# alexklwong/calibrated-backprojection-network

Hardware: AMD Instinct MI355X
Metric: depth-completion frames/sec at 352x1216 (higher is better)
Workload: dtype f32; 1 GPU; KITTI 352x1216, batch 32/GPU, fp32, full KBNet forward in HIP, random xavier weights; frames_per_gpu=32, global_batch=32, height=352, width=1216, n_ranks_seen=1, collective_backend=nccl, gathered_frames=32, launch=HIP graph replay, 2 concurrent sub-batch branch(es)

## Files before the change

### calibrated-backprojection-network_amd/_lib.py

```python

from __future__ import annotations

import ctypes as C
import os

import torch

HERE = os.path.dirname(os.path.abspath(__file__))
LIB_PATH = os.environ.get("KBN_LIB_PATH") or os.path.join(HERE, "libkbnet_hip.so")

KBN_OK = 0
KBN_ERR_INVALID_ARGUMENT, KBN_ERR_UNSUPPORTED, KBN_ERR_WORKSPACE, KBN_ERR_LAUNCH = -1, -2, -3, -4
KBN_SRC_TENSOR, KBN_SRC_COORDS, KBN_SRC_XYZ, KBN_SRC_PAIR = 0, 1, 2, 3
KBN_ACT_ELU, KBN_ACT_SIGMOID = 1, 2
KBN_RESIZE_NONE, KBN_RESIZE_NEAREST = 0, 1
KBN_MAX_SRC = 3
KBN_ADAM_TABLE_CAPACITY, KBN_ADAM_PASS_ELEMENTS = 48, 524288
KBN_MULTI_COPY_TABLE_CAPACITY, KBN_MULTI_COPY_PASS_ELEMENTS = 48, 524288
KBN_AUGMENT_ROLE_IMAGE, KBN_AUGMENT_ROLE_RANGE, KBN_AUGMENT_ROLE_VALIDITY = 0, 1, 2
KBN_AUGMENT_RANGE_0_255, KBN_AUGMENT_RANGE_0_1, KBN_AUGMENT_RANGE_M1_1 = 0, 1, 2
KBN_AUGMENT_NOISE_NONE, KBN_AUGMENT_NOISE_GAUSSIAN, KBN_AUGMENT_NOISE_UNIFORM = 0, 1, 2
KBN_AUGMENT_STAGE_SELECT, KBN_AUGMENT_STAGE_APPLY = 1, 2
KBN_AUGMENT_MAX_FRAMES, KBN_AUGMENT_WORKSPACE_RECORD_BYTES = 512, 16
KBN_UNPACK_TRAIN_MAX_FRAMES = 64
# ... 202 lines not shown
    "kbn_add_act_backward": (_I, [_P, _P, _P, _L, _I, _F, _P]),
    "kbn_resize_nearest_forward": (_I, [_P, _L, _P, _L, _I, _I, _I, _I, _I, _I, _P]),
    "kbn_resize_nearest_backward": (_I, [_P, _L, _P, _L, _I, _I, _I, _I, _I, _I, _P]),
    "kbn_kb_xyz_backward": (_I, [_P, _L, _P, _L, _P, _L, _P, _L, _I, _I, _I, _I, _F, _P]),
    "kbn_depth_map_backward": (_I, [_P, _P, _P, _P, _L, _F, _P]),
    "kbn_depth_head_forward": (_I, [_P, _P, _P, _P, _I, _I, _I, _I, _F, _F, _P]),
    "kbn_conv_head_forward": (_I, [_P, _L, _P, _P, _P, _P, _I, _I, _I, _I, _I, _F, _F, _F, _P]),
    "kbn_conv_tail_packed_weight_bytes": (C.c_size_t, [_I]),
    "kbn_conv_tail_pack_weight": (_I, [_P, _P, _I, _P]),
    "kbn_conv_tail_forward": (_I, [_P, _L, _P, _P, _P, _P, _I, _I, _I, _I, _I, _F, _F, _F, _P]),
    "kbn_conv_tail_forward_pair": (_I, [_P, _L, _P, _P, _P, _P, _P, _I, _I, _I, _I, _I, _F, _F, _F, _P]),
    "kbn_absmax_frames": (_I, [_P, _L, _I, _L, _P, _P]),
    "kbn_conv3x3_split_packed_weight_bytes": (C.c_size_t, [_I, _I, _I]),
    "kbn_conv3x3_split_pack_weight": (_I, [_P, _P, _I, _I, _I, _P]),
    "kbn_conv3x3_split_forward": (_I, [C.POINTER(ConvSrc), _I, _P, _P, _L, _I, _I, _I, _I, _I, _I, _I, _F, _P, _P, _L, _P, _P]),
    "kbn_conv3x3_split_forward_ksplit": (_I, [C.POINTER(ConvSrc), _I, _P, _P, _L, _I, _I, _I, _I, _I, _I, _I, _F, _P, _I, _P, _P]),
    "kbn_conv1x1s2_split_packed_weight_bytes": (C.c_size_t, [_I, _I, _I]),
    "kbn_conv1x1s2_split_pack_weight": (_I, [_P, _P, _I, _I, _I, _P]),
    "kbn_conv1x1s2_split_forward": (_I, [C.POINTER(ConvSrc), _I, _P, _P, _L, _P, _L, _I, _I, _I, _I, _I, _I, _F, _P, _P]),
    "kbn_kb_xyz_s2_forward": (_I, [_P, _L, _I, _I, _I, _P, _P, _I, _F, _P, _L, _I, _P]),
    "kbn_adam_step": (_I, [C.POINTER(AdamTensor), _I, _P]),
    "kbn_multi_tensor_scale_copy": (_I, [C.POINTER(CopyTensor), _I, _F, _P]),
    "kbn_augment_workspace_bytes": (C.c_size_t, [C.POINTER(AugmentTensor), _I, _I, _I, _I]),
    "kbn_augment_forward": (_I, [C.POINTER(AugmentTensor), _I, C.c_char_p, _I, _I, _I, _P, _P, C.c_size_t, _I, _I, _F, C.c_ulonglong, C.c_uint, _I, _P]),
    "kbn_augment_forward_at": (_I, [C.POINTER(AugmentTensor), _I, C.c_char_p, _I, _I, _I, _P, _P, C.c_size_t, _I, _I, _F, C.c_ulonglong, C.c_uint, C.c_uint, _I, _P]),
    "kbn_summary_panel_forward": (_I, [C.POINTER(SummaryRow), _I, _I, _I, _I, _F, _P, _P]),
    "kbn_summary_colorize_forward": (_I, [_P, _L, _L, _L, _I, _I, _I, _I, _P, _P]),
    "kbn_png_info": (_I, [_P, C.c_size_t, _P, _P, _P, _P]),
    "kbn_png_decode": (_I, [_P, C.c_size_t, _P, C.c_size_t]),
    "kbn_png_decode_batch": (_I, [_P, _P, _P, _P, _I, _I, _P]),
# ... 60 lines not shown
```

### calibrated-backprojection-network_amd/csrc/abi.hip

```cpp
#include <stdlib.h>
#include <string.h>

#include "kbn_common.h"

namespace kbn {

KnobValue g_knobs[KNOB_COUNT];

static const char* const kKnobNames[KNOB_COUNT] = {
    "KBN_DEBUG", "KBN_FORCE_MW", "KBN_FORCE_TWB", "KBN_EPI_LDS", "KBN_NO_WINO",
    "KBN_NO_UP2X9", "KBN_NO_UP2X3", "KBN_WINO_RT",
    "KBN_NO_KB_PAIR", "KBN_NO_KB_DEPTH_FUSION", "KBN_PAIR_CAND", "KBN_S2D_DEBUG", "KBN_AUTOTUNE",
    "KBN_NO_HEAD_FUSION", "KBN_NO_SPLIT", "KBN_NO_OVERLAP", "KBN_NO_PAIR", "KBN_NO_PAIR_MID", "KBN_NO_PAIR_ENC",
    "KBN_NO_PAIR_TAIL", "KBN_NO_DEPTH_FRONT_FUSION", "KBN_FP16_ONE_TERM", "KBN_DEPTH_FRONT_FUSION", "KBN_NO_FRONT_NEXT"};

void tune_reload_env();

static void load_knobs() {
    for (int k = 0; k < KNOB_COUNT; ++k) {
        const char* v = getenv(kKnobNames[k]);
        g_knobs[k].set = (v && *v) ? 1 : 0;
        int val = 0;
        if (v && *v) {
            char* end = nullptr;
            const long parsed = strtol(v, &end, 10);
            val = (end == v) ? 1 : (int)parsed;
        }
        g_knobs[k].value = val;
    }
// ... 51 lines not shown
```

### calibrated-backprojection-network_amd/csrc/conv_split.hip

```cpp
#include "split_common.h"

#ifndef KBN_SPLIT_PRIO
#define KBN_SPLIT_PRIO 0
#endif

namespace kbn {

__global__ void split_scale_kernel(const float* __restrict__ w, float* __restrict__ inv_scale, int OC, int per_filter) {
    const int oc = blockIdx.x;
    __shared__ float red[256];
    float m = 0.f;
    if (oc < OC)
        for (int i = threadIdx.x; i < per_filter; i += 256) m = fmaxf(m, fabsf(w[(long long)oc * per_filter + i]));
    red[threadIdx.x] = m;
    __syncthreads();
    for (int s = 128; s > 0; s >>= 1) {
        if (threadIdx.x < s) red[threadIdx.x] = fmaxf(red[threadIdx.x], red[threadIdx.x + s]);
        __syncthreads();
    }
    if (threadIdx.x == 0) {
        int ex = SP_WEXP;
        if (red[0] > 0.f && red[0] < 3.0e38f) (void)frexpf(red[0], &ex);
        int e = SP_WEXP - ex;
        e = e > 100 ? 100 : (e < -100 ? -100 : e);
// ... 176 lines not shown
                       reinterpret_cast<float*>(static_cast<unsigned char*>(packed) + bytes - l1_bytes), out_channels, in_channels, 9);
    if (mode == 3) upconv_split_pack(weight, inv, wp, out_channels, in_channels, ocpad, total, tr, (hipStream_t)stream);
    else split_pack_launch(weight, inv, wp, out_channels, in_channels * 9, in_channels, nt, total, 9, in_channels, 0, (hipStream_t)stream);
    KBN_CHECK_LAUNCH();
    return KBN_OK;
}

int kbn_absmax_frames(const float* x, long long batch_stride, int n, long long per_frame, unsigned* slots, kbn_stream_t stream) {
    return kbn::absmax_frames_launch(x, batch_stride, n, per_frame, slots, (hipStream_t)stream);
}

static int conv3x3_split_impl(const kbn_conv_src* srcs, int n_src, const void* packed_weight, float* out,
                              long long out_batch_stride, int n, int out_channels, int height, int width, int mode,
                              int act_exponent, int apply_activation, float negative_slope, unsigned* out_absmax,
                              void* pair_out, long long pair_out_batch_stride, float* pair_out_scale, int ksplit, float* workspace,
                              kbn_stream_t stream) {
    using namespace kbn;
    if (act_exponent < -60 || act_exponent > 60) return KBN_ERR_INVALID_ARGUMENT;
    if (!srcs || n_src < 1 || n_src > 2 || !packed_weight || (!out && !pair_out) || n < 1 || out_channels < 1 || height < 1 || width < 1)
        return KBN_ERR_INVALID_ARGUMENT;
    if (mode == 4) mode = 3;
    if (mode < 0 || mode > 3) return KBN_ERR_INVALID_ARGUMENT;
    if (knob(KNOB_NO_SPLIT)) return KBN_ERR_UNSUPPORTED;
    const bool vec4 = pair_out || !((width & 3) || (reinterpret_cast<uintptr_t>(out) & 15) || (out_batch_stride & 3));
    if (!vec4 && (mode == 1 || mode == 3)) return KBN_ERR_UNSUPPORTED;
    if ((mode == 1 || mode == 3) && (n_src != 1 || (height & 1) || (width & 1))) return KBN_ERR_UNSUPPORTED;
    SplitConvParams p{};
    int cin = 0;
    for (int s = 0; s < n_src; ++s) {
        const kbn_conv_src& a = srcs[s];
        const bool pair = a.kind == KBN_SRC_PAIR;
// ... 33 lines not shown
    p.nTilesN = ceil_div(out_channels, ntf);
    p.inv_scale = static_cast<const float*>(packed_weight);
    p.wp = reinterpret_cast<const _Float16*>(p.inv_scale + p.nTilesN * ntf);
    p.l1 = reinterpret_cast<const float*>(static_cast<const unsigned char*>(packed_weight) +
                                          kbn_conv3x3_split_packed_weight_bytes(out_channels, cin, mode) - (size_t)(cin / SP_CK) * 4);
    if (pair_out) {
        const bool narrow = mode == 3 && uf_narrow(out_channels, cin);
        const bool kernel_ok = (mode == 0) || (mode == 3 && ntf == U64_NT && !uf_narrow(out_channels, cin)) ||
                               (mode == 2 && n_src == 1) || narrow;
        if (!kernel_ok || (!narrow && (out_channels & 7))) return KBN_ERR_UNSUPPORTED;
        const int pair_channels = narrow ? U16_NT : out_channels;
        if (!p.amax[0] || (n_src > 1 && !p.amax[1]) || !pair_out_scale || (reinterpret_cast<uintptr_t>(pair_out) & 15) ||
            (pair_out_batch_stride & 7) || pair_out_batch_stride < (long long)(pair_channels / 8) * 2 * pair_plane_halves(height, width))
            return KBN_ERR_INVALID_ARGUMENT;
        p.pair_out = static_cast<_Float16*>(pair_out); p.pair_out_bstride = pair_out_batch_stride; p.pair_out_scale = pair_out_scale;
    }
    if (p.pair_src && mode == 3 && !(ntf == U64_NT || uf_narrow(out_channels, cin))) return KBN_ERR_UNSUPPORTED;
    if (p.pair_src && mode == 3 && uf_narrow(out_channels, cin) && (srcs[0].channels % U16_CK)) return KBN_ERR_UNSUPPORTED;
    p.out = out; p.out_bstride = out_batch_stride;
    p.N = n; p.OC = out_channels; p.Cin = cin; p.H = height; p.W = width;
    p.tilesX = ceil_div(width, SP_TW); p.tilesY = ceil_div(height, mode == 2 ? SpGeom<2>::TH : SpGeom<0>::TH);
    if (mode == 3) { p.tilesX = ceil_div(p.sW, 32); p.tilesY = ceil_div(p.sH, 16); }
    const long long blocks = (long long)p.tilesX * p.tilesY * n * p.nTilesN;
    if (blocks > 0x7fffffffLL) return KBN_ERR_UNSUPPORTED;
    p.nblocks = (int)blocks;
    p.act = apply_activation ? 1 : 0; p.slope = negative_slope;
    p.prescale = ldexpf(1.f, act_exponent); p.unscale = ldexpf(1.f, -act_exponent);
    p.vec4 = vec4 ? 1 : 0;
    p.ksplit = 1;
    if (ksplit > 1) {
// ... 53 lines not shown
        }, p.pair_src != nullptr, p.pair_out != nullptr, one_term);
    }
    if (rc != KBN_OK) return rc;
    KBN_CHECK_LAUNCH();
    return KBN_OK;
}

int kbn_conv3x3_split_forward(const kbn_conv_src* srcs, int n_src, const void* packed_weight, float* out,
                              long long out_batch_stride, int n, int out_channels, int height, int width, int mode,
                              int act_exponent, int apply_activation, float negative_slope, unsigned* out_absmax,
                              void* pair_out, long long pair_out_batch_stride, float* pair_out_scale, kbn_stream_t stream) {
    return conv3x3_split_impl(srcs, n_src, packed_weight, out, out_batch_stride, n, out_channels, height, width, mode, act_exponent,
                              apply_activation, negative_slope, out_absmax, pair_out, pair_out_batch_stride, pair_out_scale, 1, nullptr, stream);
}

int kbn_conv3x3_split_forward_ksplit(const kbn_conv_src* srcs, int n_src, const void* packed_weight, float* out,
                                     long long out_batch_stride, int n, int out_channels, int height, int width, int mode,
                                     int act_exponent, int apply_activation, float negative_slope, unsigned* out_absmax,
                                     int ksplit, float* workspace, kbn_stream_t stream) {
    if (ksplit < 1) return KBN_ERR_INVALID_ARGUMENT;
    return conv3x3_split_impl(srcs, n_src, packed_weight, out, out_batch_stride, n, out_channels, height, width, mode, act_exponent,
                              apply_activation, negative_slope, out_absmax, nullptr, 0, nullptr, ksplit, workspace, stream);
}

}
```

### calibrated-backprojection-network_amd/csrc/kbn_common.h

```cpp
#pragma once

#include <hip/hip_runtime.h>
#include <stdint.h>

#include <atomic>
#include <type_traits>

#include "../../include/kbnet_hip.h"

#define KBN_CHECK_LAUNCH()                                   \
    do {                                                     \
        hipError_t e__ = hipGetLastError();                  \
        if (e__ != hipSuccess) return KBN_ERR_LAUNCH;        \
    } while (0)

namespace kbn {

typedef float f32x4 __attribute__((ext_vector_type(4)));
typedef float f32x2 __attribute__((ext_vector_type(2)));

__host__ __device__ inline int ceil_div(int a, int b) { return (a + b - 1) / b; }
__host__ __device__ inline int round_up(int a, int b) { return ceil_div(a, b) * b; }
inline bool layer_shape_ok(int out_channels, int in_channels, int kernel_size) {
    return out_channels >= 1 && in_channels >= 1 && kernel_size >= 1 && kernel_size <= 7 && out_channels <= KBN_MAX_CHANNELS &&
// ... 55 lines not shown
template <class F>
int flag_dispatch(F&& f) { return f(); }
template <class F, class... Flags>
int flag_dispatch(F&& f, bool flag, Flags... rest) {
    auto bind = [&](auto c) { return flag_dispatch([&](auto... more) { return f(c, more...); }, rest...); };
    return flag ? bind(std::true_type{}) : bind(std::false_type{});
}
int device_cu_count();

enum Knob {
    KNOB_DEBUG, KNOB_FORCE_MW, KNOB_FORCE_TWB, KNOB_EPI_LDS, KNOB_NO_WINO,
    KNOB_NO_UP2X9, KNOB_NO_UP2X3, KNOB_WINO_RT,
    KNOB_NO_KB_PAIR, KNOB_NO_KB_DEPTH_FUSION, KNOB_PAIR_CAND, KNOB_S2D_DEBUG, KNOB_AUTOTUNE,
    KNOB_NO_HEAD_FUSION, KNOB_NO_SPLIT,
    KNOB_NO_OVERLAP, KNOB_NO_PAIR, KNOB_NO_PAIR_MID, KNOB_NO_PAIR_ENC, KNOB_NO_PAIR_TAIL, KNOB_NO_DEPTH_FRONT_FUSION,
    KNOB_FP16_ONE_TERM, KNOB_DEPTH_FRONT_FUSION, KNOB_NO_FRONT_NEXT, KNOB_COUNT
};
struct KnobValue { int set, value; };
extern KnobValue g_knobs[KNOB_COUNT];
inline int knob(Knob k) { return g_knobs[k].value; }
inline bool knob_set(Knob k) { return g_knobs[k].set != 0; }

__device__ __forceinline__ int xcd_remap(int bid, int nblocks) {
    const int NX = 8;
    int xcd = bid % NX, idx = bid / NX;
    int q = nblocks / NX, r = nblocks % NX;
    int start = (xcd < r) ? xcd * (q + 1) : r * (q + 1) + (xcd - r) * q;
    return start + idx;
}

__device__ __forceinline__ int nearest_src_index(int dst, int in_size, int out_size) {
// ... 14 lines not shown
```

### calibrated-backprojection-network_amd/csrc/split_common.h

```cpp

#pragma once
#include "conv_common.h"

#include <type_traits>

#ifndef KBN_SPLIT_STRAIGHT
#define KBN_SPLIT_STRAIGHT 1
#endif

namespace kbn {

typedef _Float16 sph8 __attribute__((ext_vector_type(8)));
typedef _Float16 sph2 __attribute__((ext_vector_type(2)));
typedef float spf16 __attribute__((ext_vector_type(16)));
typedef float spf4 __attribute__((ext_vector_type(4)));
typedef _Float16 sph4 __attribute__((ext_vector_type(4)));

constexpr int SP_TW = 32, SP_CK = 16, SP_TH = 16, SP_THREADS = 512;
constexpr int SP_WEXP = 13;

template <int MODE>
struct SpGeom {
    static constexpr bool S2 = MODE == 2;
    static constexpr int TH = S2 ? 8 : SP_TH;
// ... 19 lines not shown
    int tilesX, tilesY, nTilesN, nblocks;
    int act;
    float slope;
    int vec4;
    float prescale;
    float unscale;
    const unsigned* amax[2];
    unsigned* out_amax;
    const _Float16* pair_src;
    long long pair_src_bstride;
    const float* pair_src_scale;
    _Float16* pair_out;
    long long pair_out_bstride;
    float* pair_out_scale;
    const float* l1;
    int tp_x0, tp_tilesY, tp_nblocks;
    int sub0;
    const float* xyz;
    long long xyz_bstride;
    const float* wxyz;
    int ksplit;
    long long ks_stride;
};

__device__ __forceinline__ void sp_split8(const float (&v)[8], float prescale, sph8& h1, sph8& h2) {
    const float prescale_hi = prescale * 2048.f;
#pragma unroll
    for (int k = 0; k < 8; k += 2) {
        const f32x2 a = {v[k], v[k + 1]};
        const sph2 c1 = __builtin_convertvector(a * prescale, sph2);
// ... 23 lines not shown
}


__device__ __forceinline__ float sp_scale_of_bound(float bound) {
    int k = 14 + 127 - (int)(__float_as_uint(bound) >> 23 & 255u);
    k = k > 100 ? 100 : (k < -100 ? -100 : k);
    return __uint_as_float((unsigned)(127 + k) << 23);
}
__device__ __forceinline__ float sp_pair_out_scale(const SplitConvParams& p, int n) {
    const int nchunks = p.Cin / SP_CK, n0 = p.nsrc > 1 ? p.srcC[0] / SP_CK : nchunks;
    float w0 = 0.f, w1 = 0.f;
    for (int c = 0; c < n0; ++c) w0 += p.l1[c];
    for (int c = n0; c < nchunks; ++c) w1 += p.l1[c];
    float bound = __uint_as_float(p.amax[0][n]) * w0;
    if (p.nsrc > 1) bound += __uint_as_float(p.amax[1][n]) * w1;
    return sp_scale_of_bound(bound);
}
__device__ __forceinline__ void sp_act_scale_of(const SplitConvParams& p, int s, int n, float& prescale, float& unscale) {
    prescale = p.prescale;
    unscale = p.unscale;
    if (p.amax[s]) {
        int k = 14 + 127 - (int)(p.amax[s][n] >> 23);
        k = k > 100 ? 100 : (k < -100 ? -100 : k);
        prescale = __uint_as_float((unsigned)(127 + k) << 23);
        unscale = __uint_as_float((unsigned)(127 - k) << 23);
    }
}
typedef unsigned spu2 __attribute__((ext_vector_type(2)));
typedef unsigned spu4 __attribute__((ext_vector_type(4)));
__device__ __forceinline__ spu4 sp_pair_exchange(const sph4& a, const sph4& b) {
// ... 48 lines not shown
```

### calibrated-backprojection-network_amd/modules.py

```python

from __future__ import annotations

import os
from typing import List, Optional

import torch

from . import _lib, ops, optim
from ._lib import KbnError
from .config import KBNetConfig


def activation_func(activation_fn: str):
    if "linear" in activation_fn:
        return None
    if "leaky_relu" in activation_fn:
        return torch.nn.LeakyReLU(negative_slope=0.20, inplace=True)
    if "relu" in activation_fn:
        return torch.nn.ReLU()
    if "elu" in activation_fn:
        return torch.nn.ELU()
    if "sigmoid" in activation_fn:
        return torch.nn.Sigmoid()
    raise ValueError("Unsupported activation function: {}".format(activation_fn))
# ... 55 lines not shown
        if self._blob is not None:
            self.get(*self._args[0], **self._args[1])


def packed_blobs(model):
    return [v for top in model.modules() for sub in top.modules() for v in vars(sub).values() if isinstance(v, _PackedBlob)]


def data_gradient_blob(layer, weight):
    blob = layer.__dict__.get("_packed_bwd_data")
    if blob is None:
        blob = layer._packed_bwd_data = _PackedBlob(ops.pack_conv2d_data_gradient_weight)
    return blob.get(weight, stride=layer.stride)


def _run_split(layer, weight, srcs, n, h, w, out=None, up2x=False, out_absmax=None, stats=None, pair_out=False, transposed=False):
    kinds_ok = all((s.kind == _lib.KBN_SRC_TENSOR or (i == 0 and s.kind == _lib.KBN_SRC_PAIR)) and s.channels % 16 == 0
                   for i, s in enumerate(srcs))
    if (not layer.split or layer.kernel_size != 3 or (up2x and w % 4) or len(srcs) > 2 or (up2x and layer.stride != 1)
            or not kinds_ok or (pair_out and layer._post is not None)):
        return None
    narrow_up = up2x and layer.split_narrow_up and layer.out_channels <= 16 and layer.in_channels % 32 == 0
    if layer.out_channels < 48 and not narrow_up:
        return None
    dev = weight.device
    srcs = Conv2d._with_slots(srcs, n, dev, stats)
    if pair_out:
        if stats is None or (layer.out_channels % 8 and not narrow_up) or (layer.stride != 1 and up2x):
            return None
        out = ops.PairTensor(n, 16 if narrow_up else layer.out_channels, h, w, dev, stats)
        if layer.stride == 2:
            out.with_sub()
        if out_absmax is not None:
            out.absmax = out_absmax
    elif out is None:
        out = torch.empty((n, layer.out_channels, h, w), device=dev, dtype=torch.float32)
    packed = layer._split_blob(up2x)
    ks = 1
    if getattr(layer, "latency", 0) and not pair_out and all(s.kind == _lib.KBN_SRC_TENSOR for s in srcs):
        ks = ops.ksplit_for(sum(s.channels for s in srcs), layer.out_channels, h, w, layer.stride, up2x=up2x, frames=layer.latency)
    kw = dict(up2x=up2x, negative_slope=layer._slope, stride=layer.stride, folded_up2x=up2x, out_absmax=None if layer._post else out_absmax,
              transposed=transposed)
    res = ops.conv3x3_split(srcs, packed, n, layer.out_channels, h, w, out, ksplit=ks, **kw) if ks > 1 else None
    if res is None:
        res = ops.conv3x3_split(srcs, packed, n, layer.out_channels, h, w, out, **kw)
    return res if res is None else _finish(layer, res, out_absmax)


class Conv2d(torch.nn.Module):

    def __init__(self, in_channels, out_channels, kernel_size=3, stride=1,
                 weight_initializer="kaiming_uniform",
                 activation_func=torch.nn.LeakyReLU(negative_slope=0.10, inplace=True),
                 use_batch_norm=False, use_instance_norm=False):
        super().__init__()
        if use_batch_norm or use_instance_norm:
            raise ValueError("normalisation layers are not part of the KBNet inference path")
# ... 19 lines not shown
    def _with_slots(srcs, n, dev, stats):
        for s in srcs:
            if s.kind == _lib.KBN_SRC_TENSOR and (not s.absmax or (stats is not None and not stats.usable(s.absmax))):
                if stats is None:
                    stats = ops.ActStats(n, dev, capacity=len(srcs))
                slot = stats.measure(s._keep[0])
                s.absmax = slot.data_ptr()
                s._keep = (s._keep[0], slot)
        return srcs

    def _split_blob(self, up2x):
        if up2x:
            return self._packed_split_up.get(self.conv.weight, folded_up2x=True)
        return self._packed_split.get(self.conv.weight, stride=self.stride)

    def run_split(self, srcs, n, h, w, out=None, up2x=False, out_absmax=None, stats=None, pair_out=False):
        return _run_split(self, self.conv.weight, srcs, n, h, w, out, up2x, out_absmax, stats, pair_out)

    def split_fused_qualifies(self, ci, cf):
        return (self.split and self.kernel_size == 1 and self.stride == 2 and ci % 16 == 0 and cf % 16 == 0
                and self.out_channels >= self.split_fused_min_filters and self.in_channels == ci + 3 + cf)

    def run_split_fused(self, image, fused, xyz, n, h, w, out, amax_image=None, amax_fused=None, out_absmax=None, stats=None):
        ci, cf = image.shape[1], (0 if fused is None else fused.shape[1])
        if not self.split_fused_qualifies(ci, cf):
            return None
        if isinstance(image, ops.PairTensor):
            if image.sub is None or fused is None:
                return None
            image, amax_image = image.sub, image.absmax
        srcs = [ops.tensor_src(image, "image", amax_image)] + ([] if fused is None else [ops.tensor_src(fused, "fused", amax_fused)])
        srcs = self._with_slots(srcs, n, image.device, stats)
# ... 424 lines not shown
                parts = [ops.s2d_pyramid(x, mins[i:i + 8], []) for i in range(0, len(mins), 8)]
                parts += [ops.s2d_pyramid(x, [], maxs[i:i + 8]) for i in range(0, len(maxs), 8)]
                y = torch.cat(parts, dim=1)
            for conv in self.pool_convs:
                y = conv.run([ops.tensor_src(y, "pool")], n, h, w)
            return self.conv.run([ops.tensor_src(y, "pool"), ops.tensor_src(x, "x")], n, h, w)
        return ops.s2d_forward(x, [c.conv.weight for c in self.pool_convs], self.conv.conv.weight,
                               self.min_pool_sizes, self.max_pool_sizes, self._slope)


class KBNetEncoder(torch.nn.Module):

    pair_chain = _KnobSwitch("KBN_NO_PAIR", "KBN_NO_PAIR_ENC")
    fuse_s2d = _KnobSwitch("KBN_NO_DEPTH_FRONT_FUSION", enable="KBN_DEPTH_FRONT_FUSION")
    front_next = _KnobSwitch("KBN_NO_FRONT_NEXT")

    def __init__(self, input_channels_image=3, input_channels_depth=1,
                 n_filters_image=[48, 96, 192, 384, 384], n_filters_depth=[16, 32, 64, 128, 128],
                 n_filters_fused=[48, 96, 192, 384, 384], n_convolutions_image=[1, 1, 1, 1, 1],
                 n_convolutions_depth=[1, 1, 1, 1, 1], n_convolutions_fused=[1, 1, 1, 1, 1],
                 resolutions_backprojection=[0, 1, 2], weight_initializer="kaiming_uniform",
                 activation_func="leaky_relu"):
        super().__init__()
        for lst in (n_convolutions_image, n_convolutions_depth, n_convolutions_fused, n_filters_image,
                    n_filters_depth, n_filters_fused):
            assert len(lst) == 5
        if 0 not in resolutions_backprojection:
            raise ValueError("resolution 0 must use calibrated backprojection (undefined in the reference otherwise)")
        self.resolutions_backprojection = list(resolutions_backprojection)
        act = globals()["activation_func"](activation_func)
# ... 99 lines not shown
            raise KbnError("kb1_front declined a problem kbn_kb1_front_query accepted")
        return skip, out_image, out_depth, out_fused, a_img, a_skip, nxt_info

    def _image_splitk(self, level, h, w):
        blk = getattr(self, f"calibrated_backprojection{level + 1}", None)
        if blk is None:
            return False
        ci = blk.conv_image.conv_block[0]
        frames = getattr(ci, "latency", 0)
        return bool(frames) and ops.ksplit_for(ci.in_channels, ci.out_channels, (h + 1) // 2, (w + 1) // 2, 2, frames=frames) > 1

    def forward(self, image, depth, intrinsics):
        latent, skips, _, _ = self.encode(image, depth, intrinsics)
        return latent, skips

    def encode(self, image, depth, intrinsics, stats=None, s2d=None):
        fi, fd, ff = self._f
        n, _, h0, w0 = image.shape
        if stats is None:
            stats = ops.ActStats(n, image.device)
        dev = image.device
        image = image if _dense(image) else image.contiguous()
        if depth is not None:
            depth = depth if _dense(depth) else depth.contiguous()
        intrinsics = intrinsics.contiguous()

        kinv = ops.intrinsics_inverse(intrinsics, 1.0, 1.0)
        h, w = h0, w0
        h1, w1 = (h0 + 1) // 2, (w0 + 1) // 2
        sx, sy = w1 / w0, h1 / h0
        kinv1_box = []
# ... 65 lines not shown
            amax_skips.append(a_skip)
            h, w = oh, ow
        oh, ow = (h + 1) // 2, (w + 1) // 2
        amax_latent = stats.new()
        if 4 in self.resolutions_backprojection:
            if 3 not in self.resolutions_backprojection:
                raise AttributeError("'KBNetEncoder' object has no attribute 'calibrated_backprojection4'")
            blk = self.calibrated_backprojection4
            if isinstance(conv_image, ops.PairTensor):
                conv_image, amax_image = conv_image.float(), None
            latent = torch.empty((n, blk.n_filter_fused + blk.n_filter_depth, oh, ow), device=dev, dtype=torch.float32)
            blk.run(conv_image, conv_depth, kinv1_get(), conv_fused, None, latent[:, blk.n_filter_fused:], latent[:, :blk.n_filter_fused],
                    amax_image=amax_image, amax_fused=amax_skip if conv_fused is not None else None, out_amax_image=stats.new(),
                    out_amax_skip=amax_latent, stats=stats, need_image=not self.skip_unused_image)
            return latent, skips, amax_latent, amax_skips
        latent = torch.empty((n, fi[4] + fd[4], oh, ow), device=dev, dtype=torch.float32)
        src, a_src = (conv_fused, amax_skip) if conv_fused is not None else (conv_image, amax_image)
        branch = _SideBranch(dev)
        self.conv5_image.run([ops.tensor_src(src, "image", a_src)], n, h, w, out=latent[:, :fi[4]],
                             out_absmax=amax_latent, stats=stats)
        with branch:
            self.conv5_depth.run([ops.tensor_src(conv_depth, "depth", amax_skip)], n, h, w, out=latent[:, fi[4]:],
                                 out_absmax=amax_latent, stats=stats)
        return latent, skips, amax_latent, amax_skips


class MultiScaleDecoder(torch.nn.Module):

    pair_chain = _KnobSwitch("KBN_NO_PAIR")
    pair_tail = _KnobSwitch("KBN_NO_PAIR_TAIL")

    def __init__(self, input_channels=256, output_channels=1, n_resolution=1,
# ... 3 lines not shown
        super().__init__()
        if n_resolution != 1 or output_func != "linear" or len(n_filters) != 5 or output_channels != 1:
            raise ValueError("implemented for KBNet's decoder: 5 levels, n_resolution=1, linear 1-channel output")
        if use_batch_norm or use_instance_norm:
            raise ValueError("normalisation layers are not part of the KBNet inference path")
        self.n_resolution = n_resolution
        self.output_func = output_func
        act = globals()["activation_func"](activation_func)
        cin = input_channels
        for i, name in enumerate(("deconv4", "deconv3", "deconv2", "deconv1", "deconv0")):
            setattr(self, name, DecoderBlock(cin, n_skips[i], n_filters[i], weight_initializer, act,
                                             deconv_type=deconv_type))
            cin = n_filters[i]
        self.output0 = Conv2d(n_filters[4], output_channels, 3, 1, weight_initializer, None)
        self._packed_tail = _PackedBlob(ops.pack_conv_tail_weight)

    def features(self, x, skips, shape):
        stats = ops.ActStats(x.shape[0], x.device)
        x, amax = self.features_level1(x, skips, stats=stats)
        return self.deconv0(x, None, shape=tuple(shape)[-2:], amax_x=amax, stats=stats)

    def features_level1(self, x, skips, amax_x=None, amax_skips=None, stats=None, allow_pair=False):
        if stats is None:
            stats = ops.ActStats(x.shape[0], x.device)
        amax_skips = amax_skips if amax_skips is not None else [None] * 4
        amax = amax_x
        for blk, i in ((self.deconv4, 3), (self.deconv3, 2), (self.deconv2, 1), (self.deconv1, 0)):
            a_out = stats.new()
            y = None
            if not isinstance(x, ops.PairTensor) and blk.latency_splitk(x.shape[2], x.shape[3]):
# ... 234 lines not shown
        if return_inner:
            raise KbnError("KBNetModel.forward: return_inner exists on the recorded path only (trainable=True, grad mode on, a parameter "
                           "that requires grad): the fused forward never materialises most activations")
        return self._forward_fused(image, sparse_depth, validity_map_depth, intrinsics, return_logits, out)

    @torch.no_grad()
    def _forward_fused(self, image, sparse_depth, validity_map_depth, intrinsics, return_logits=False, out=None):
        if out is not None and return_logits:
            raise KbnError("out= and return_logits are mutually exclusive")
        input_depth = paired_planes(sparse_depth, validity_map_depth)
        if input_depth is None:
            input_depth = torch.cat([sparse_depth, validity_map_depth], dim=1)
        shape = input_depth.shape[-2:]
        stats = ops.ActStats(image.shape[0], image.device)
        latent, skips, amax_latent, amax_skips = self.encoder.encode(image, None, intrinsics, stats,
                                                                     s2d=(self.sparse_to_dense_pool, input_depth.contiguous()))
        return self.decoder.depth(latent, skips, shape, self.min_predict_depth, self.max_predict_depth,
                                  return_logits=return_logits, out=out, amax_x=amax_latent, amax_skips=amax_skips, stats=stats)

    def set_latency_mode(self, enabled: bool = True, frames: int = 1):
        frames = int(frames) if enabled else 0
        if enabled and frames < 1:
            raise KbnError("set_latency_mode: frames must be at least 1")
        for top in self.modules():
            for m in top.modules():
                if isinstance(m, (Conv2d, TransposeConv2d)):
                    m.latency = frames
        self.latency_mode = frames
        return self

    def capture(self, image, sparse_depth, validity_map_depth, intrinsics, branches=None, tune=True, outputs=1, split_graphs=False):
# ... 85 lines not shown
```

### calibrated-backprojection-network_amd/ops.py

```python

from __future__ import annotations

import contextlib
import ctypes as C
import functools
import struct
from typing import List, Optional, Sequence

import torch

from . import _lib
from ._lib import ConvSrc, KbnError, check


def _stream() -> int:
    return torch.cuda.current_stream().cuda_stream


def _on_tensor_device(fn):
    @functools.wraps(fn)
    def wrapper(*args, **kwargs):
        idx = None
        for a in list(args) + list(kwargs.values()):
            if isinstance(a, torch.Tensor) and a.is_cuda:
# ... 300 lines not shown
            PairTensor.LOG.append(self)
        self.shape = (n, channels, height, width)
        self.data = torch.empty((n, channels // 8, 2, height * width + 1, 8), device=device, dtype=torch.float16)
        self.scale = torch.empty(n, device=device, dtype=torch.float32)
        self.absmax = stats.new()
        self.sub: Optional[torch.Tensor] = None

    @property
    def device(self):
        return self.data.device

    def with_sub(self) -> "PairTensor":
        n, c, h, w = self.shape
        self.sub = torch.empty((n, c, (h + 1) // 2, (w + 1) // 2), device=self.data.device, dtype=torch.float32)
        return self

    def window_slack_log2(self) -> torch.Tensor:
        amax = slot_values(self.absmax).double().clamp_min(1e-300)
        return 15.0 - torch.log2(amax * self.scale.double())

    def float(self) -> torch.Tensor:
        n, c, h, w = self.shape
        v = self.data[:, :, 0, :h * w].double() + self.data[:, :, 1, :h * w].double() / 2048.0
        v = v / self.scale.double().view(n, 1, 1, 1)
        return v.permute(0, 1, 3, 2).reshape(n, c, h, w).float()


def pair_src(t: PairTensor, name="src") -> ConvSrc:
    n, c, h, w = t.shape
    s = ConvSrc()
# ... 318 lines not shown
            px = sh * 32 * (sw // 32) + -(-sh // 2) * 32
        else:
            px = sh * (-(-sw // seg) * seg)
        return 3 * 2.0 * n * px * cin * 16 * (-(-out_channels // nblk) * nblk)
    if stride == 1 and width >= 32 and 1 <= width % 32 <= 16:
        px = height * 32 * (width // 32) + -(-height // 2) * 32
    else:
        px = height * (-(-width // 32) * 32)
    return 3 * 2.0 * n * px * cin * 9 * (-(-out_channels // 32) * 32)


@_on_tensor_device
def conv3x3_split(srcs: List[ConvSrc], packed_weight: torch.Tensor, n: int, out_channels: int, height: int, width: int,
                  out: torch.Tensor, up2x: bool = False, negative_slope: Optional[float] = 0.2, stride: int = 1,
                  act_exponent: int = -6, folded_up2x: bool = False, out_absmax: Optional[torch.Tensor] = None,
                  transposed: bool = False, ksplit: int = 1):
    if transposed and not (up2x and folded_up2x):
        raise KbnError("conv3x3_split: transposed goes with up2x and folded_up2x")
    if up2x and stride != 1:
        raise KbnError("conv3x3_split: up2x and stride 2 are mutually exclusive")
    lib = _lib.load()
    arr = (ConvSrc * len(srcs))(*srcs)
    pair = isinstance(out, PairTensor)
    if pair:
        optr, obs = (None, 0) if (out.sub is None or stride != 2) else _planes(out.sub, "out.sub")
        if out_absmax is None:
            out_absmax = out.absmax
    else:
        optr, obs = _planes(out, "out")
    want = (n, 16 if (pair and up2x and folded_up2x and out_channels <= 16) else out_channels, height, width)
    if tuple(out.shape) != want:
        raise KbnError(f"out has shape {tuple(out.shape)}, expected {want}")
    cin = sum(s.channels for s in srcs)
    flops = 2.0 * n * height * width * cin * 9 * out_channels / (4 if transposed else 1)
    mode = (4 if transposed else (3 if folded_up2x else 1)) if up2x else (2 if stride == 2 else 0)
    if ksplit > 1:
        if pair or mode == 1:
            raise KbnError("conv3x3_split: ksplit goes with the plain / stride-2 / folded up-conv forms and an fp32 output")
        ws = torch.empty((ksplit, n, out_channels, height, width), device=out.device, dtype=torch.float32)
        done = _launched("kbn_conv3x3_split_forward_ksplit", ("conv_split", "", "conv_split_s2", "conv_split_upfold", "conv_split_upfold")[mode], flops,
                         lambda: lib.kbn_conv3x3_split_forward_ksplit(arr, len(srcs), packed_weight.data_ptr(), optr, obs, n, out_channels, height, width,
                                                                      mode, max(-60, min(60, int(act_exponent))), *_act_args(negative_slope),
                                                                      _slot_ptr(out_absmax, n), int(ksplit), ws.data_ptr(), _stream()),
                         executed=conv3x3_split_executed_flops(n, cin, out_channels, height, width, stride, up2x and folded_up2x),
                         pipe="fp16", nbytes=_src_bytes(srcs, n) + 4.0 * n * height * width * out_channels * (1 + 2 * ksplit))
        return out if done else None
    if not _launched("kbn_conv3x3_split_forward", ("conv_split", "conv_split_up", "conv_split_s2", "conv_split_upfold", "conv_split_upfold")[mode], flops,
                     lambda: lib.kbn_conv3x3_split_forward(arr, len(srcs), packed_weight.data_ptr(), optr, obs, n,
                                                           out_channels, height, width,
                                                           mode, max(-60, min(60, int(act_exponent))),
# ... 2119 lines not shown
```

### include/kbnet_hip.h

```cpp
#ifndef KBNET_HIP_H
#define KBNET_HIP_H

#include <stddef.h>

#ifdef __cplusplus
extern "C" {
#endif

#define KBN_ABI_VERSION 11

typedef void* kbn_stream_t;

typedef enum kbn_status {
    KBN_OK = 0,
    KBN_ERR_INVALID_ARGUMENT = -1,
    KBN_ERR_UNSUPPORTED = -2,
    KBN_ERR_WORKSPACE = -3,
    KBN_ERR_LAUNCH = -4
} kbn_status;

int kbn_version(void);
const char* kbn_status_string(int status);

void kbn_reload_env(void);
// ... 82 lines not shown

int kbn_deconv2x_pack_weight(const float* weight, float* packed, int out_channels, int in_channels,
                             kbn_stream_t stream);
int kbn_deconv2x_forward(const float* src, long long src_batch_stride, const float* packed_weight,
                         float* out, long long out_batch_stride, int n, int in_channels,
                         int out_channels, int src_height, int src_width, int apply_activation,
                         float negative_slope, unsigned* out_absmax, kbn_stream_t stream);

size_t kbn_conv3x3_split_packed_weight_bytes(int out_channels, int in_channels, int mode);
int kbn_conv3x3_split_pack_weight(const float* weight, void* packed, int out_channels, int in_channels, int mode,
                                  kbn_stream_t stream);
int kbn_conv3x3_split_forward(const kbn_conv_src* srcs, int n_src, const void* packed_weight, float* out,
                              long long out_batch_stride, int n, int out_channels, int height, int width, int mode,
                              int act_exponent, int apply_activation, float negative_slope, unsigned* out_absmax,
                              void* pair_out, long long pair_out_batch_stride, float* pair_out_scale, kbn_stream_t stream);
int kbn_conv3x3_split_forward_ksplit(const kbn_conv_src* srcs, int n_src, const void* packed_weight, float* out,
                                     long long out_batch_stride, int n, int out_channels, int height, int width, int mode,
                                     int act_exponent, int apply_activation, float negative_slope, unsigned* out_absmax,
                                     int ksplit, float* workspace, kbn_stream_t stream);

size_t kbn_conv1x1s2_split_packed_weight_bytes(int out_channels, int tensor_channels, int has_xyz);
int kbn_conv1x1s2_split_pack_weight(const float* weight, void* packed, int out_channels, int in_channels, int xyz_offset,
                                    kbn_stream_t stream);
int kbn_conv1x1s2_split_forward(const kbn_conv_src* srcs, int n_src, const void* packed_weight, const float* xyz,
                                long long xyz_batch_stride, float* out, long long out_batch_stride, int n, int out_channels,
                                int height, int width, int act_exponent, int apply_activation, float negative_slope,
                                unsigned* out_absmax, kbn_stream_t stream);
int kbn_kb_xyz_s2_forward(const float* depth, long long depth_batch_stride, int depth_channels, int height, int width,
                          const float* proj_weight, const float* kinv, int apply_activation, float negative_slope, float* xyz,
                          long long xyz_batch_stride, int n, kbn_stream_t stream);
// ... 360 lines not shown
```

Baseline: 3069 frames/s.

## Emit encoder latent as shared-scale fp16 pair tensor from both conv5 branches

The conv5 image and depth convolutions now write straight into one fp16 PairTensor latent, each into its own channel range. To make that possible they share one quantisation scale: each kernel's bound also takes in the peer branch's weight L1 norms and activation absmax. This drops the fp32 latent write and the later conversion into pair form for the decoder's first up-convolution. In exchange the scale computation grows, precision may drop for the branch with the smaller range, and many eligibility checks gate the path.

```diff
diff --git a/calibrated-backprojection-network_amd/_lib.py b/calibrated-backprojection-network_amd/_lib.py
--- a/calibrated-backprojection-network_amd/_lib.py
+++ b/calibrated-backprojection-network_amd/_lib.py
@@ -240,6 +240,8 @@
     "kbn_conv3x3_split_packed_weight_bytes": (C.c_size_t, [_I, _I, _I]),
     "kbn_conv3x3_split_pack_weight": (_I, [_P, _P, _I, _I, _I, _P]),
     "kbn_conv3x3_split_forward": (_I, [C.POINTER(ConvSrc), _I, _P, _P, _L, _I, _I, _I, _I, _I, _I, _I, _F, _P, _P, _L, _P, _P]),
+    "kbn_conv3x3_split_forward_shared": (_I, [C.POINTER(ConvSrc), _I, _P, _P, _L, _I, _I, _I, _I, _I, _I, _I, _F, _P, _P, _L, _P,
+                                               _P, _I, _I, _I, _P, _P]),
     "kbn_conv3x3_split_forward_ksplit": (_I, [C.POINTER(ConvSrc), _I, _P, _P, _L, _I, _I, _I, _I, _I, _I, _I, _F, _P, _I, _P, _P]),
     "kbn_conv1x1s2_split_packed_weight_bytes": (C.c_size_t, [_I, _I, _I]),
     "kbn_conv1x1s2_split_pack_weight": (_I, [_P, _P, _I, _I, _I, _P]),
diff --git a/calibrated-backprojection-network_amd/csrc/abi.hip b/calibrated-backprojection-network_amd/csrc/abi.hip
--- a/calibrated-backprojection-network_amd/csrc/abi.hip
+++ b/calibrated-backprojection-network_amd/csrc/abi.hip
@@ -12,7 +12,8 @@
     "KBN_NO_UP2X9", "KBN_NO_UP2X3", "KBN_WINO_RT",
     "KBN_NO_KB_PAIR", "KBN_NO_KB_DEPTH_FUSION", "KBN_PAIR_CAND", "KBN_S2D_DEBUG", "KBN_AUTOTUNE",
     "KBN_NO_HEAD_FUSION", "KBN_NO_SPLIT", "KBN_NO_OVERLAP", "KBN_NO_PAIR", "KBN_NO_PAIR_MID", "KBN_NO_PAIR_ENC",
-    "KBN_NO_PAIR_TAIL", "KBN_NO_DEPTH_FRONT_FUSION", "KBN_FP16_ONE_TERM", "KBN_DEPTH_FRONT_FUSION", "KBN_NO_FRONT_NEXT"};
+    "KBN_NO_PAIR_TAIL", "KBN_NO_DEPTH_FRONT_FUSION", "KBN_FP16_ONE_TERM", "KBN_DEPTH_FRONT_FUSION", "KBN_NO_FRONT_NEXT",
+    "KBN_NO_PAIR_SKIP"};
 
 void tune_reload_env();
 
diff --git a/calibrated-backprojection-network_amd/csrc/conv_split.hip b/calibrated-backprojection-network_amd/csrc/conv_split.hip
--- a/calibrated-backprojection-network_amd/csrc/conv_split.hip
+++ b/calibrated-backprojection-network_amd/csrc/conv_split.hip
@@ -214,7 +214,7 @@
                               long long out_batch_stride, int n, int out_channels, int height, int width, int mode,
                               int act_exponent, int apply_activation, float negative_slope, unsigned* out_absmax,
                               void* pair_out, long long pair_out_batch_stride, float* pair_out_scale, int ksplit, float* workspace,
-                              kbn_stream_t stream) {
+                              kbn_stream_t stream, const float* peer_l1 = nullptr, int peer_chunks = 0, const unsigned* peer_absmax = nullptr) {
     using namespace kbn;
     if (act_exponent < -60 || act_exponent > 60) return KBN_ERR_INVALID_ARGUMENT;
     if (!srcs || n_src < 1 || n_src > 2 || !packed_weight || (!out && !pair_out) || n < 1 || out_channels < 1 || height < 1 || width < 1)
@@ -278,6 +278,9 @@
             (pair_out_batch_stride & 7) || pair_out_batch_stride < (long long)(pair_channels / 8) * 2 * pair_plane_halves(height, width))
             return KBN_ERR_INVALID_ARGUMENT;
         p.pair_out = static_cast<_Float16*>(pair_out); p.pair_out_bstride = pair_out_batch_stride; p.pair_out_scale = pair_out_scale;
+        p.peer_l1 = peer_l1; p.peer_chunks = peer_chunks; p.peer_amax = peer_absmax;
+    } else if (peer_l1) {
+        return KBN_ERR_INVALID_ARGUMENT;
     }
     if (p.pair_src && mode == 3 && !(ntf == U64_NT || uf_narrow(out_channels, cin))) return KBN_ERR_UNSUPPORTED;
     if (p.pair_src && mode == 3 && uf_narrow(out_channels, cin) && (srcs[0].channels % U16_CK)) return KBN_ERR_UNSUPPORTED;
@@ -361,6 +364,22 @@
                               apply_activation, negative_slope, out_absmax, pair_out, pair_out_batch_stride, pair_out_scale, 1, nullptr, stream);
 }
 
+int kbn_conv3x3_split_forward_shared(const kbn_conv_src* srcs, int n_src, const void* packed_weight, float* out,
+                                     long long out_batch_stride, int n, int out_channels, int height, int width, int mode,
+                                     int act_exponent, int apply_activation, float negative_slope, unsigned* out_absmax,
+                                     void* pair_out, long long pair_out_batch_stride, float* pair_out_scale,
+                                     const void* peer_packed_weight, int peer_out_channels, int peer_in_channels, int peer_mode,
+                                     const unsigned* peer_absmax, kbn_stream_t stream) {
+    if (!pair_out || n_src != 1 || !peer_packed_weight || !peer_absmax) return KBN_ERR_INVALID_ARGUMENT;
+    const size_t peer_bytes = kbn_conv3x3_split_packed_weight_bytes(peer_out_channels, peer_in_channels, peer_mode);
+    if (peer_bytes == 0) return KBN_ERR_INVALID_ARGUMENT;
+    const int peer_chunks = peer_in_channels / kbn::SP_CK;
+    const float* peer_l1 = reinterpret_cast<const float*>(static_cast<const unsigned char*>(peer_packed_weight) + peer_bytes - (size_t)peer_chunks * 4);
+    return conv3x3_split_impl(srcs, n_src, packed_weight, out, out_batch_stride, n, out_channels, height, width, mode, act_exponent,
+                              apply_activation, negative_slope, out_absmax, pair_out, pair_out_batch_stride, pair_out_scale, 1, nullptr, stream,
+                              peer_l1, peer_chunks, peer_absmax);
+}
+
 int kbn_conv3x3_split_forward_ksplit(const kbn_conv_src* srcs, int n_src, const void* packed_weight, float* out,
                                      long long out_batch_stride, int n, int out_channels, int height, int width, int mode,
                                      int act_exponent, int apply_activation, float negative_slope, unsigned* out_absmax,
diff --git a/calibrated-backprojection-network_amd/csrc/kbn_common.h b/calibrated-backprojection-network_amd/csrc/kbn_common.h
--- a/calibrated-backprojection-network_amd/csrc/kbn_common.h
+++ b/calibrated-backprojection-network_amd/csrc/kbn_common.h
@@ -93,7 +93,7 @@
     KNOB_NO_KB_PAIR, KNOB_NO_KB_DEPTH_FUSION, KNOB_PAIR_CAND, KNOB_S2D_DEBUG, KNOB_AUTOTUNE,
     KNOB_NO_HEAD_FUSION, KNOB_NO_SPLIT,
     KNOB_NO_OVERLAP, KNOB_NO_PAIR, KNOB_NO_PAIR_MID, KNOB_NO_PAIR_ENC, KNOB_NO_PAIR_TAIL, KNOB_NO_DEPTH_FRONT_FUSION,
-    KNOB_FP16_ONE_TERM, KNOB_DEPTH_FRONT_FUSION, KNOB_NO_FRONT_NEXT, KNOB_COUNT
+    KNOB_FP16_ONE_TERM, KNOB_DEPTH_FRONT_FUSION, KNOB_NO_FRONT_NEXT, KNOB_NO_PAIR_SKIP, KNOB_COUNT
 };
 struct KnobValue { int set, value; };
 extern KnobValue g_knobs[KNOB_COUNT];
diff --git a/calibrated-backprojection-network_amd/csrc/split_common.h b/calibrated-backprojection-network_amd/csrc/split_common.h
--- a/calibrated-backprojection-network_amd/csrc/split_common.h
+++ b/calibrated-backprojection-network_amd/csrc/split_common.h
@@ -57,6 +57,9 @@
     long long pair_out_bstride;
     float* pair_out_scale;
     const float* l1;
+    const float* peer_l1;
+    int peer_chunks;
+    const unsigned* peer_amax;
     int tp_x0, tp_tilesY, tp_nblocks;
     int sub0;
     const float* xyz;
@@ -110,6 +113,11 @@
     for (int c = n0; c < nchunks; ++c) w1 += p.l1[c];
     float bound = __uint_as_float(p.amax[0][n]) * w0;
     if (p.nsrc > 1) bound += __uint_as_float(p.amax[1][n]) * w1;
+    if (p.peer_l1) {
+        float wp = 0.f;
+        for (int c = 0; c < p.peer_chunks; ++c) wp += p.peer_l1[c];
+        bound = fmaxf(bound, __uint_as_float(p.peer_amax[n]) * wp);
+    }
     return sp_scale_of_bound(bound);
 }
 __device__ __forceinline__ void sp_act_scale_of(const SplitConvParams& p, int s, int n, float& prescale, float& unscale) {
diff --git a/calibrated-backprojection-network_amd/modules.py b/calibrated-backprojection-network_amd/modules.py
--- a/calibrated-backprojection-network_amd/modules.py
+++ b/calibrated-backprojection-network_amd/modules.py
@@ -93,7 +93,7 @@
     return blob.get(weight, stride=layer.stride)
 
 
-def _run_split(layer, weight, srcs, n, h, w, out=None, up2x=False, out_absmax=None, stats=None, pair_out=False, transposed=False):
+def _run_split(layer, weight, srcs, n, h, w, out=None, up2x=False, out_absmax=None, stats=None, pair_out=False, transposed=False, peer=None):
     kinds_ok = all((s.kind == _lib.KBN_SRC_TENSOR or (i == 0 and s.kind == _lib.KBN_SRC_PAIR)) and s.channels % 16 == 0
                    for i, s in enumerate(srcs))
     if (not layer.split or layer.kernel_size != 3 or (up2x and w % 4) or len(srcs) > 2 or (up2x and layer.stride != 1)
@@ -107,11 +107,12 @@
     if pair_out:
         if stats is None or (layer.out_channels % 8 and not narrow_up) or (layer.stride != 1 and up2x):
             return None
-        out = ops.PairTensor(n, 16 if narrow_up else layer.out_channels, h, w, dev, stats)
-        if layer.stride == 2:
-            out.with_sub()
-        if out_absmax is not None:
-            out.absmax = out_absmax
+        if not isinstance(out, ops.PairTensor):
+            out = ops.PairTensor(n, 16 if narrow_up else layer.out_channels, h, w, dev, stats)
+            if layer.stride == 2:
+                out.with_sub()
+            if out_absmax is not None:
+                out.absmax = out_absmax
     elif out is None:
         out = torch.empty((n, layer.out_channels, h, w), device=dev, dtype=torch.float32)
     packed = layer._split_blob(up2x)
@@ -120,6 +121,8 @@
         ks = ops.ksplit_for(sum(s.channels for s in srcs), layer.out_channels, h, w, layer.stride, up2x=up2x, frames=layer.latency)
     kw = dict(up2x=up2x, negative_slope=layer._slope, stride=layer.stride, folded_up2x=up2x, out_absmax=None if layer._post else out_absmax,
               transposed=transposed)
+    if peer is not None:
+        kw["peer"] = peer
     res = ops.conv3x3_split(srcs, packed, n, layer.out_channels, h, w, out, ksplit=ks, **kw) if ks > 1 else None
     if res is None:
         res = ops.conv3x3_split(srcs, packed, n, layer.out_channels, h, w, out, **kw)
@@ -169,8 +172,8 @@
             return self._packed_split_up.get(self.conv.weight, folded_up2x=True)
         return self._packed_split.get(self.conv.weight, stride=self.stride)
 
-    def run_split(self, srcs, n, h, w, out=None, up2x=False, out_absmax=None, stats=None, pair_out=False):
-        return _run_split(self, self.conv.weight, srcs, n, h, w, out, up2x, out_absmax, stats, pair_out)
+    def run_split(self, srcs, n, h, w, out=None, up2x=False, out_absmax=None, stats=None, pair_out=False, peer=None):
+        return _run_split(self, self.conv.weight, srcs, n, h, w, out, up2x, out_absmax, stats, pair_out, peer=peer)
 
     def split_fused_qualifies(self, ci, cf):
         return (self.split and self.kernel_size == 1 and self.stride == 2 and ci % 16 == 0 and cf % 16 == 0
@@ -625,6 +628,7 @@
     pair_chain = _KnobSwitch("KBN_NO_PAIR", "KBN_NO_PAIR_ENC")
     fuse_s2d = _KnobSwitch("KBN_NO_DEPTH_FRONT_FUSION", enable="KBN_DEPTH_FRONT_FUSION")
     front_next = _KnobSwitch("KBN_NO_FRONT_NEXT")
+    pair_latent = _KnobSwitch("KBN_NO_PAIR", "KBN_NO_PAIR_SKIP")
 
     def __init__(self, input_channels_image=3, input_channels_depth=1,
                  n_filters_image=[48, 96, 192, 384, 384], n_filters_depth=[16, 32, 64, 128, 128],
@@ -754,7 +758,32 @@
         latent, skips, _, _ = self.encode(image, depth, intrinsics)
         return latent, skips
 
-    def encode(self, image, depth, intrinsics, stats=None, s2d=None):
+    def _pair_latent(self, src, a_src, conv_depth, a_depth, n, h, w, oh, ow, amax_latent, stats):
+        ci, cd = self.conv5_image.conv_block, self.conv5_depth.conv_block
+        if len(ci) != 1 or len(cd) != 1 or not ops.split_enabled():
+            return None
+        ci, cd = ci[0], cd[0]
+        for c in (ci, cd):
+            if (not c.split or c.kernel_size != 3 or c.stride != 2 or c._post is not None or c.out_channels < 48 or c.out_channels % 8
+                    or c.in_channels % 16 or getattr(c, "latency", 0)):
+                return None
+        dev = src.device
+        s_img = Conv2d._with_slots([ops.tensor_src(src, "image", a_src)], n, dev, stats)
+        s_dep = Conv2d._with_slots([ops.tensor_src(conv_depth, "depth", a_depth)], n, dev, stats)
+        latent = ops.PairTensor(n, ci.out_channels + cd.out_channels, oh, ow, dev, stats)
+        latent.absmax = amax_latent
+        peer_of = lambda c, s: (c._split_blob(False), c.out_channels, c.in_channels, c.stride, s[0]._keep[1])
+        branch = _SideBranch(dev)
+        res = ci.run_split(s_img, n, oh, ow, out=latent.channel_range(0, ci.out_channels), out_absmax=amax_latent, stats=stats,
+                           pair_out=True, peer=peer_of(cd, s_dep))
+        if res is None:
+            return None
+        with branch:
+            res = cd.run_split(s_dep, n, oh, ow, out=latent.channel_range(ci.out_channels, ci.out_channels + cd.out_channels),
+                               out_absmax=amax_latent, stats=stats, pair_out=True, peer=peer_of(ci, s_img))
+        return latent if res is not None else None
+
+    def encode(self, image, depth, intrinsics, stats=None, s2d=None, pair_latent=False):
         fi, fd, ff = self._f
         n, _, h0, w0 = image.shape
         if stats is None:
@@ -850,8 +879,12 @@
                     amax_image=amax_image, amax_fused=amax_skip if conv_fused is not None else None, out_amax_image=stats.new(),
                     out_amax_skip=amax_latent, stats=stats, need_image=not self.skip_unused_image)
             return latent, skips, amax_latent, amax_skips
+        src, a_src = (conv_fused, amax_skip) if conv_fused is not None else (conv_image, amax_image)
+        if pair_latent and self.pair_latent:
+            latent = self._pair_latent(src, a_src, conv_depth, amax_skip, n, h, w, oh, ow, amax_latent, stats)
+            if latent is not None:
+                return latent, skips, amax_latent, amax_skips
         latent = torch.empty((n, fi[4] + fd[4], oh, ow), device=dev, dtype=torch.float32)
-        src, a_src = (conv_fused, amax_skip) if conv_fused is not None else (conv_image, amax_image)
         branch = _SideBranch(dev)
         self.conv5_image.run([ops.tensor_src(src, "image", a_src)], n, h, w, out=latent[:, :fi[4]],
                              out_absmax=amax_latent, stats=stats)
@@ -885,6 +918,18 @@
             cin = n_filters[i]
         self.output0 = Conv2d(n_filters[4], output_channels, 3, 1, weight_initializer, None)
         self._packed_tail = _PackedBlob(ops.pack_conv_tail_weight)
+
+    def takes_pair_latent(self, shape):
+        up = self.deconv4.deconv.conv if isinstance(self.deconv4.deconv, UpConv2d) else self.deconv4.deconv
+        oc = up.out_channels
+        def size(v, levels):
+            for _ in range(levels):
+                v = (int(v) + 1) // 2
+            return v
+        exact = all(size(v, 4) == 2 * size(v, 5) for v in shape[-2:])
+        return bool(self.pair_chain and up.split and getattr(self.deconv4.deconv, "split_up", True) and up._post is None
+                    and oc >= 64 and (-(-oc // 32)) % 2 == 0 and up.in_channels % 16 == 0 and not getattr(up, "latency", 0)
+                    and exact and size(shape[-1], 4) % 4 == 0)
 
     def features(self, x, skips, shape):
         stats = ops.ActStats(x.shape[0], x.device)
@@ -1149,7 +1194,8 @@
         shape = input_depth.shape[-2:]
         stats = ops.ActStats(image.shape[0], image.device)
         latent, skips, amax_latent, amax_skips = self.encoder.encode(image, None, intrinsics, stats,
-                                                                     s2d=(self.sparse_to_dense_pool, input_depth.contiguous()))
+                                                                     s2d=(self.sparse_to_dense_pool, input_depth.contiguous()),
+                                                                     pair_latent=self.decoder.takes_pair_latent(shape))
         return self.decoder.depth(latent, skips, shape, self.min_predict_depth, self.max_predict_depth,
                                   return_logits=return_logits, out=out, amax_x=amax_latent, amax_skips=amax_skips, stats=stats)
 
diff --git a/calibrated-backprojection-network_amd/ops.py b/calibrated-backprojection-network_amd/ops.py
--- a/calibrated-backprojection-network_amd/ops.py
+++ b/calibrated-backprojection-network_amd/ops.py
@@ -338,6 +338,16 @@
         n, c, h, w = self.shape
         self.sub = torch.empty((n, c, (h + 1) // 2, (w + 1) // 2), device=self.data.device, dtype=torch.float32)
         return self
+
+    def channel_range(self, c0: int, c1: int) -> "PairTensor":
+        n, c, h, w = self.shape
+        if c0 % 8 or c1 % 8 or not 0 <= c0 < c1 <= c:
+            raise KbnError(f"PairTensor.channel_range: {c0}:{c1} of {c} channels is not a range of whole k-groups")
+        v = object.__new__(PairTensor)
+        v.shape = (n, c1 - c0, h, w)
+        v.data = self.data[:, c0 // 8:c1 // 8]
+        v.scale, v.absmax, v.sub = self.scale, self.absmax, None
+        return v
 
     def window_slack_log2(self) -> torch.Tensor:
         amax = slot_values(self.absmax).double().clamp_min(1e-300)
@@ -686,7 +696,7 @@
 def conv3x3_split(srcs: List[ConvSrc], packed_weight: torch.Tensor, n: int, out_channels: int, height: int, width: int,
                   out: torch.Tensor, up2x: bool = False, negative_slope: Optional[float] = 0.2, stride: int = 1,
                   act_exponent: int = -6, folded_up2x: bool = False, out_absmax: Optional[torch.Tensor] = None,
-                  transposed: bool = False, ksplit: int = 1):
+                  transposed: bool = False, ksplit: int = 1, peer: Optional[tuple] = None):
     if transposed and not (up2x and folded_up2x):
         raise KbnError("conv3x3_split: transposed goes with up2x and folded_up2x")
     if up2x and stride != 1:
@@ -706,6 +716,20 @@
     cin = sum(s.channels for s in srcs)
     flops = 2.0 * n * height * width * cin * 9 * out_channels / (4 if transposed else 1)
     mode = (4 if transposed else (3 if folded_up2x else 1)) if up2x else (2 if stride == 2 else 0)
+    if peer is not None:
+        if not pair or ksplit > 1 or len(srcs) != 1 or up2x:
+            raise KbnError("conv3x3_split: peer goes with a PairTensor output, one source and the plain or stride-2 form")
+        p_packed, p_oc, p_cin, p_stride, p_absmax = peer
+        if not _launched("kbn_conv3x3_split_forward_shared", ("conv_split", "", "conv_split_s2")[mode], flops,
+                         lambda: lib.kbn_conv3x3_split_forward_shared(arr, len(srcs), packed_weight.data_ptr(), optr, obs, n, out_channels, height, width,
+                                                                      mode, max(-60, min(60, int(act_exponent))), *_act_args(negative_slope),
+                                                                      _slot_ptr(out_absmax, n), out.data.data_ptr(), out.data.stride(0), out.scale.data_ptr(),
+                                                                      p_packed.data_ptr(), int(p_oc), int(p_cin), 2 if p_stride == 2 else 0,
+                                                                      _slot_ptr(p_absmax, n), _stream()),
+                         executed=conv3x3_split_executed_flops(n, cin, out_channels, height, width, stride, False),
+                         pipe="fp16", nbytes=_src_bytes(srcs, n) + 4.0 * n * height * width * out_channels):
+            return None
+        return out
     if ksplit > 1:
         if pair or mode == 1:
             raise KbnError("conv3x3_split: ksplit goes with the plain / stride-2 / folded up-conv forms and an fp32 output")
diff --git a/include/kbnet_hip.h b/include/kbnet_hip.h
--- a/include/kbnet_hip.h
+++ b/include/kbnet_hip.h
@@ -120,6 +120,12 @@
                               long long out_batch_stride, int n, int out_channels, int height, int width, int mode,
                               int act_exponent, int apply_activation, float negative_slope, unsigned* out_absmax,
                               void* pair_out, long long pair_out_batch_stride, float* pair_out_scale, kbn_stream_t stream);
+int kbn_conv3x3_split_forward_shared(const kbn_conv_src* srcs, int n_src, const void* packed_weight, float* out,
+                                     long long out_batch_stride, int n, int out_channels, int height, int width, int mode,
+                                     int act_exponent, int apply_activation, float negative_slope, unsigned* out_absmax,
+                                     void* pair_out, long long pair_out_batch_stride, float* pair_out_scale,
+                                     const void* peer_packed_weight, int peer_out_channels, int peer_in_channels, int peer_mode,
+                                     const unsigned* peer_absmax, kbn_stream_t stream);
 int kbn_conv3x3_split_forward_ksplit(const kbn_conv_src* srcs, int n_src, const void* packed_weight, float* out,
                                      long long out_batch_stride, int n, int out_channels, int height, int width, int mode,
                                      int act_exponent, int apply_activation, float negative_slope, unsigned* out_absmax,
```

New measurement: 3053 frames/s. No clear change (-0.5%).
